# dream-faster/laplace-gnn-recommendation

Measured on AMD Instinct MI355X. Metric: positive-edges/sec (train step), higher is better.
Workload: dtype f32; 1 GPU; LightGCN train step, ONE synthetic bipartite graph 8000000x100000 users x items, 100000000 edges (seed 3, 64 user blocks), sharded by user over 1 GPU(s): 8000000 users / 100000000 edges per GPU, 3-layer D=128, global batch 131072 positive edges, on-device sampling, BPR + dense Adam; BASELINE.json configs[3]; parallelism=1 GPU

## Files before the change

### include/laplace_hip.h

```cpp
#ifndef LAPLACE_HIP_H
#define LAPLACE_HIP_H

#include <stddef.h>
#include <stdint.h>

#ifdef __cplusplus
extern "C" {
#endif

#define MI_ABI_VERSION 14

#define MI_ERR_BAD_ARG      (-1)
#define MI_ERR_TOO_LARGE    (-2)
#define MI_ERR_WORKSPACE    (-3)
#define MI_ERR_UNSUPPORTED  (-4)

typedef void* mi_stream_t;

int         mi_abi_version(void);
const char* mi_error_string(int code);

size_t mi_coo_to_csr_workspace_bytes(int64_t n_rows, int64_t nnz);
int    mi_coo_to_csr_i32(int64_t n_rows, int64_t n_cols, int64_t nnz,
                         const int64_t* row, const int64_t* col,
// ... 54 lines not shown
                               mi_spmm_plan_info* info, mi_stream_t stream);
int    mi_spmm_plan_fill(int64_t n_rows, const int32_t* rowptr, const mi_spmm_plan_info* info,
                         mi_spmm_plan* plan, void* ws, size_t ws_bytes, mi_stream_t stream);
size_t mi_spmm_plan_pack_workspace_bytes(int64_t n_launch);
int    mi_spmm_plan_pack_entries(const mi_spmm_plan* plan, int64_t nnz_long, const int32_t* col, const float* val,
                                 int32_t values_only, void* ws, size_t ws_bytes, mi_stream_t stream);
size_t mi_spmm_workspace_bytes(const mi_spmm_plan* plan, int64_t d);

int mi_spmm_csr_f32(int64_t n_rows, int64_t d,
                    const int32_t* rowptr, const int32_t* col, const float* val,
                    const float* X, int64_t ldx,
                    float* Y, int64_t ldy,
                    const float* addend, int64_t lda,
                    float* S, int64_t lds, float scale,
                    const mi_spmm_plan* plan, void* ws, size_t ws_bytes,
                    mi_stream_t stream);

typedef struct mi_adam_args {
    float*       p;  int64_t ldp;
    float*       m;
    float*       v;
    const float* reg_w;
    double       lr, beta1, beta2, eps;
    int64_t      step;
} mi_adam_args;

typedef struct mi_spmm_sweep {
    const int32_t* col;
    const float*   val;
    const int32_t* stream_ptr;
    const int32_t* slot_of;
    int32_t        n_streams;
    int32_t        n_slots;
    int32_t*       progress;
    int32_t        epoch;
    int32_t        slack;
} mi_spmm_sweep;

typedef struct mi_spmm_ex {
    const int32_t* x_map;
    const int32_t* addend_map;
    const int32_t* row_list;
    const int32_t* n_list_dev;
    int64_t        n_list;
    const mi_adam_args* adam;
    int32_t        parts;
    int32_t        hot_rows;
    const mi_spmm_sweep* sweep;
    int32_t        hot_base;
    int32_t        hot_threads;
    const uint32_t* x_bits;
    const int32_t* thin_rows;
    int32_t        n_thin;
} mi_spmm_ex;
#define MI_SPMM_SHORT_ROWS 1
#define MI_SPMM_SPLIT_ROWS 2

int mi_spmm_csr_ex_f32(int64_t n_rows, int64_t d,
                       const int32_t* rowptr, const int32_t* col, const float* val,
                       const float* X, int64_t ldx,
                       float* Y, int64_t ldy,
                       const float* addend, int64_t lda,
                       float* S, int64_t lds, float scale,
                       const mi_spmm_plan* plan, const mi_spmm_ex* ex,
                       void* ws, size_t ws_bytes, mi_stream_t stream);

int mi_map_live_bits_i32(int64_t n, const int32_t* map, uint32_t* bits, mi_stream_t stream);

int mi_gather_rows_f32(int64_t n_max, const int32_t* n_dev, const int32_t* begin_dev, int64_t d,
                       const int32_t* rows, int64_t row_offset, const float* src, int64_t ld_src,
                       float* dst, int64_t ld_dst, int32_t accumulate, float scale,
                       mi_stream_t stream);

int mi_scatter_rows_f32(int64_t n_max, const int32_t* n_dev, const int32_t* begin_dev, int64_t d,
                        const int32_t* rows, int64_t row_offset, const float* src, int64_t ld_src,
                        float* dst, int64_t ld_dst, mi_stream_t stream);

size_t mi_batch_nodes_workspace_bytes(int64_t n_nodes);
int    mi_batch_nodes_i32(int64_t batch, int64_t n_users, int64_t n_nodes,
                          const int64_t* users, const int64_t* pos, const int64_t* neg,
                          int32_t* gmap, int32_t* nodes, int32_t* count,
                          void* ws, size_t ws_bytes, mi_stream_t stream);

#define MI_SAMPLE_KEY_COLLISION 1
#define MI_SAMPLE_NO_SELF_LOOPS 2
int mi_csr_expand_rows(int64_t n_rows, const int32_t* rowptr, int32_t* row_of_edge,
                       int64_t nnz, mi_stream_t stream);
int mi_sample_bpr_batch(int64_t batch, int64_t nnz,
                        const int32_t* rowptr, const int32_t* col,
                        const int32_t* row_of_edge,
                        int64_t neg_range, int32_t quirk_user_rows, int32_t edges_in_order,
                        uint64_t seed, uint64_t step,
                        int64_t* users, int64_t* pos, int64_t* neg,
                        mi_stream_t stream);

size_t mi_bpr_workspace_bytes(int64_t batch);
int    mi_bpr_fwd_bwd_f32(int64_t batch, int64_t d, int64_t n_users,
                          const int64_t* users, const int64_t* pos, const int64_t* neg,
                          const float* final_emb, int64_t ldf,
                          const float* e0, int64_t lde,
                          float lambda, float g_scale, float reg_scale,
                          float* loss_out,
                          float* g_final, int64_t ldg,
                          float* reg_w,
                          const int32_t* node_map,
                          void* ws, size_t ws_bytes, mi_stream_t stream);
// ... 467 lines not shown
```

### laplace-gnn-recommendation_amd/_lib.py

```python
from __future__ import annotations

import ctypes
import os
from ctypes import POINTER, Structure, c_char_p, c_double, c_float, c_int32, c_int64, c_size_t, c_uint32, c_uint64, c_void_p

PKG_DIR = os.path.dirname(os.path.abspath(__file__))
LIB_PATH = os.environ.get("LAPLACE_HIP_LIB") or os.path.join(PKG_DIR, "liblaplace_hip.so")

MI_ABI_VERSION = 14
MI_SPMM_GROUP = 32


class MiError(RuntimeError):
    pass


class SpmmPlanStruct(Structure):
    _fields_ = [
        ("chunk", c_int32), ("n_long_rows", c_int32), ("n_items", c_int32), ("n_launch", c_int32),
        ("long_rows", c_void_p), ("item_ptr", c_void_p), ("items", c_void_p), ("long_index", c_void_p),
        ("band", c_int32), ("n_bands", c_int32),
        ("epos", c_void_p), ("ecol", c_void_p), ("eval", c_void_p),
    ]


class SpmmPlanInfo(Structure):
    _fields_ = [("n_long_rows", c_int64), ("n_items", c_int64), ("n_launch", c_int64), ("nnz_long", c_int64),
                ("chunk", c_int32), ("band", c_int32), ("n_bands", c_int32), ("queue_len", c_int32),
                ("queue_start", c_int32 * 9), ("keys_in_second", c_int32)]


class AdamArgs(Structure):
    _fields_ = [("p", c_void_p), ("ldp", c_int64), ("m", c_void_p), ("v", c_void_p), ("reg_w", c_void_p),
                ("lr", c_double), ("beta1", c_double), ("beta2", c_double), ("eps", c_double), ("step", c_int64)]


class SpmmSweepStruct(Structure):
    _fields_ = [("col", c_void_p), ("val", c_void_p), ("stream_ptr", c_void_p), ("slot_of", c_void_p),
                ("n_streams", c_int32), ("n_slots", c_int32), ("progress", c_void_p), ("epoch", c_int32), ("slack", c_int32)]


class SpmmExStruct(Structure):
    _fields_ = [("x_map", c_void_p), ("addend_map", c_void_p), ("row_list", c_void_p), ("n_list_dev", c_void_p),
                ("n_list", c_int64), ("adam", POINTER(AdamArgs)), ("parts", c_int32), ("hot_rows", c_int32),
                ("sweep", POINTER(SpmmSweepStruct)), ("hot_base", c_int32), ("hot_threads", c_int32),
                ("x_bits", c_void_p), ("thin_rows", c_void_p), ("n_thin", c_int32)]


MI_SPMM_SHORT_ROWS, MI_SPMM_SPLIT_ROWS = 1, 2
MI_ERR_UNSUPPORTED = -4
MI_ERR_BAD_ARG = -1
MI_ERR_TOO_LARGE = -2
MI_ERR_WORKSPACE = -3
MI_TOPK_ITEMS_PREPARED = 1
MI_RECENT_MAX_SLOTS = 16
MI_TOPK_MERGE_MAX_ENTRIES = 4096
MI_TOPK_PATH_MATERIALISED, MI_TOPK_PATH_ONE_PASS, MI_TOPK_PATH_FUSED, MI_TOPK_PATH_FUSED_DMA, MI_TOPK_PATH_PREFILTER = range(5)
MI_RANK_OBJECTIVES = {"reference": 0, "bpr": 1, "softmax": 2}
MI_RANK_MAX_NEG = 16
MI_COOC_WEIGHTINGS = {"count": 0, "cosine": 1}


class GemmProblem(Structure):
    _fields_ = [("trans_a", c_int32), ("trans_b", c_int32), ("m", c_int64), ("n", c_int64), ("k", c_int64),
                ("A", c_void_p), ("lda", c_int64), ("B", c_void_p), ("ldb", c_int64),
                ("k2", c_int64), ("A2", c_void_p), ("lda2", c_int64), ("B2", c_void_p), ("ldb2", c_int64),
                ("a_mask", c_void_p), ("bias", c_void_p), ("C", c_void_p), ("ldc", c_int64),
                ("accumulate", c_int32), ("act", c_int32)]


class SamplerDesc(Structure):
    _fields_ = [("batch", c_int32), ("n_hops", c_int32), ("num_neighbors", c_int32), ("k", c_int32),
                ("randomization", c_int32), ("max_pos", c_int32), ("max_neg", c_int32), ("reserved", c_int32),
                ("num_users", c_int64), ("num_articles", c_int64), ("num_edges", c_int64), ("id_max", c_int64),
                ("users_ptr", c_void_p), ("users_idx", c_void_p), ("articles_ptr", c_void_p), ("articles_idx", c_void_p),
                ("positive_edges_ratio", c_double), ("negative_edges_ratio", c_double), ("reject_min_entries", c_int64),
                ("cand_ptr", c_void_p), ("cand_idx", c_void_p)]


MI_SAMPLER_MAX_RELATIONS = 4


class SamplerRelation(Structure):
    _fields_ = [("rel_ptr", c_void_p), ("rel_idx", c_void_p), ("n_targets", c_int64)]


class SamplerRelationOut(Structure):
    _fields_ = [("t_ids", c_void_p), ("t_ptr", c_void_p), ("edge3", c_void_p), ("article_rowptr", c_void_p),
                ("article_col", c_void_p), ("t_rowptr", c_void_p), ("t_col", c_void_p), ("t_cursor", c_void_p)]


MI_RANKER_MAX_LAYERS, MI_RANKER_MAX_COLS, MI_RANKER_MAX_PARAMS = 4, 16, 48


class RankerConv(Structure):
    _fields_ = [("w_l", c_void_p), ("b_l", c_void_p), ("w_r", c_void_p), ("gw_l", c_void_p), ("gb_l", c_void_p), ("gw_r", c_void_p),
                ("c_src", c_int32), ("c_dst", c_int32), ("c_out", c_int32), ("reserved", c_int32)]


# ... 316 lines not shown
```

### laplace-gnn-recommendation_amd/csrc/spmm.hip

```cpp
#include "common.hpp"
#include "pairs.hpp"
#include <algorithm>
#include <rocprim/rocprim.hpp>

namespace {

#ifndef MI_SPMM_UNROLL
#define MI_SPMM_UNROLL 4
#endif
#ifndef MI_SPMM_UNROLL_ADAM
#define MI_SPMM_UNROLL_ADAM 8
#endif
#ifndef MI_SPMM_UNROLL_PAIR
#define MI_SPMM_UNROLL_PAIR 8
#endif
#ifndef MI_SPMM_ROWS_RPS
#define MI_SPMM_ROWS_RPS 1
#endif
#ifndef MI_SPMM_NT
#define MI_SPMM_NT 0
#endif
typedef float mi_f4v __attribute__((ext_vector_type(4)));
#ifndef MI_SPMM_SC1
#define MI_SPMM_SC1 6
#endif
template <int BIT>
__device__ __forceinline__ void mi_store4(float4* p, const float4& v, bool streaming) {
    if (((MI_SPMM_SC1 >> BIT) & 1) && streaming) {
        mi_f4v x = {v.x, v.y, v.z, v.w};
        asm volatile("global_store_dwordx4 %0, %1, off sc1\n\ts_nop 1" : : "v"(p), "v"(x) : "memory");
    } else if ((MI_SPMM_NT >> BIT) & 1) {
        mi_f4v x = {v.x, v.y, v.z, v.w};
        __builtin_nontemporal_store(x, reinterpret_cast<mi_f4v*>(p));
    } else {
        *p = v;
    }
}
template <int BIT>
__device__ __forceinline__ float4 mi_load4(const float4* p) {
    if ((MI_SPMM_NT >> BIT) & 1) {
        mi_f4v x = __builtin_nontemporal_load(reinterpret_cast<const mi_f4v*>(p));
        return make_float4(x.x, x.y, x.z, x.w);
    }
    return *p;
}
#ifndef MI_SPMM_FIXUP_UNROLL
#define MI_SPMM_FIXUP_UNROLL 32
#endif
constexpr int kWavesPerBlock = 4;
constexpr int kBlock = kWavesPerBlock * MI_WAVE;
constexpr int kPlanGroup = MI_SPMM_GROUP;

struct Epilogue {
    float4* Y;            int64_t ldy4;
    const float4* addend; int64_t lda4;
    float4* S;            int64_t lds4;
    float scale;
    bool streaming;
    float4* p;            int64_t ldp4;
    float4* m;
    float4* v;
    const float* reg_w;
    MiAdamConsts adam;
};

struct Ex {
    const int32_t* x_map;
    const int32_t* addend_map;
    const int32_t* row_list;
    const int32_t* n_list_dev;
    const int32_t* long_index;
    int32_t parts;
    int32_t hot_base, hot_rows, hot_threads;
    const uint32_t* x_bits;
    uint8_t* slot_live;
    const int32_t* thin_rows;
    int32_t n_thin;
};

template <int LPR>
__device__ __forceinline__ int wave_max_over_subgroups(int n) {
#pragma unroll
    for (int m = MI_WAVE / 2; m >= LPR; m >>= 1) n = max(n, __shfl_xor(n, m, MI_WAVE));
    return n;
}

template <int LPR, int VPL, int UNROLL, bool SPARSE>
__device__ __forceinline__ void subgroup_accumulate(const int32_t* __restrict__ col,
                                                    const float* __restrict__ val,
                                                    const float4* __restrict__ X4, int64_t ldx4, int d4,
                                                    int32_t beg, int n, int nmax, int li,
                                                    const int32_t* __restrict__ x_map, float4 (&acc)[VPL]) {
    static_assert(LPR % UNROLL == 0, "a batch of LPR entries is consumed UNROLL at a time");
#pragma unroll
    for (int v = 0; v < VPL; ++v) acc[v] = mi_f4_zero();
    for (int base = 0; base < nmax; base += LPR) {
        int32_t my_c = -1;
        float my_v = 0.f;
        if (base + li < n) {
            if (MI_SPMM_NT & 1) {
                my_c = __builtin_nontemporal_load(col + beg + base + li);
                my_v = __builtin_nontemporal_load(val + beg + base + li);
            } else {
                my_c = col[beg + base + li];
                my_v = val[beg + base + li];
            }
            if (SPARSE && x_map) my_c = x_map[my_c];
        }
        if (SPARSE && __ballot(my_c >= 0) == 0ull) continue;
        const int m = min(LPR, nmax - base);
        for (int j = 0; j < m; j += UNROLL) {
            float w[UNROLL];
            float4 x[UNROLL][VPL];
#pragma unroll
            for (int u = 0; u < UNROLL; ++u) {
                const int32_t c = __shfl(my_c, j + u, LPR);
                w[u] = __shfl(my_v, j + u, LPR);
                const bool ok = c >= 0;
                const float4* src = X4 + (int64_t)(ok ? c : 0) * ldx4;
#pragma unroll
                for (int v = 0; v < VPL; ++v) {
                    const int e = li + v * LPR;
                    x[u][v] = (ok && e < d4) ? src[e] : mi_f4_zero();
                }
                if (!ok) w[u] = 0.f;
            }
#pragma unroll
            for (int u = 0; u < UNROLL; ++u)
#pragma unroll
                for (int v = 0; v < VPL; ++v) mi_f4_fma(acc[v], w[u], x[u][v]);
// ... 84 lines not shown
        if (mine) {
            r = listed ? (int64_t)ex.row_list[i] : i;
            beg = rowptr[r];
            n = rowptr[r + 1] - beg;
            mine = n <= chunk;
        }
        if (kCoop && coop && mine && n > MI_SPMM_COOP_MIN) {
            if (li == 0) {
                const int q = atomicAdd(&coop_n, 1);
                coop_row[q] = r;
                coop_beg[q] = beg;
                coop_len[q] = n;
            }
            mine = false;
        }
        if (!mine) n = 0;
        const int nmax = wave_max_over_subgroups<LPR>(n);
        float4 a[VPL], acc[VPL];
        const int64_t ar = !mine ? -1 : (listed ? i : (ex.addend_map ? (int64_t)ex.addend_map[r] : r));
        load_addend<LPR, VPL>(ep, ar, d4, li, a);
        subgroup_accumulate<LPR, VPL, UNROLL, SPARSE>(col, val, X4, ldx4, d4, beg, n, nmax, li, ex.x_map, acc);
        if (mine) store_epilogue<LPR, VPL, ADAM>(ep, listed ? i : r, d4, li, acc, a);
    }
    if (kCoop && coop) {
        __syncthreads();
        const int n_long = coop_n;
        for (int q = 0; q < n_long; ++q) {
            const int32_t beg = coop_beg[q], len = coop_len[q];
            const int64_t r = coop_row[q];
            const int32_t per = (len + SG - 1) / SG;
            const int32_t b = min(sgi * per, len);
            const int n = min(per, len - b);
            const int nmax = wave_max_over_subgroups<LPR>(n);
            float4 acc[VPL];
            subgroup_accumulate<LPR, VPL, UNROLL, false>(col, val, X4, ldx4, d4, beg + b, n, nmax, li, nullptr, acc);
#pragma unroll
            for (int v = 0; v < VPL; ++v) coop_red[sgi][v][li] = acc[v];
            __syncthreads();
            if (sgi == 0) {
                float4 a[VPL];
                load_addend<LPR, VPL>(ep, ex.addend_map ? (int64_t)ex.addend_map[r] : r, d4, li, a);
#pragma unroll
                for (int v = 0; v < VPL; ++v) {
                    float4 t = coop_red[0][v][li];
                    for (int g = 1; g < SG; ++g) t = mi_f4_add(t, coop_red[g][v][li]);
                    acc[v] = t;
                }
                store_epilogue<LPR, VPL, ADAM>(ep, r, d4, li, acc, a);
            }
            __syncthreads();
        }
    }
}
template <int LPR, int VPL, int UNROLL, int RPS, bool SPARSE, bool ADAM>
__global__ __launch_bounds__(kBlock) void spmm_rows_kernel(int64_t n_out, int d4,
                                                           const int32_t* __restrict__ rowptr,
                                                           const int32_t* __restrict__ col,
                                                           const float* __restrict__ val,
                                                           const float4* __restrict__ X4, int64_t ldx4,
                                                           Epilogue ep, int32_t chunk, Ex ex, int32_t coop) {
    spmm_rows_body<LPR, VPL, UNROLL, RPS, SPARSE, ADAM>(blockIdx.x, gridDim.x, n_out, d4, rowptr, col, val, X4, ldx4, ep, chunk, ex, coop);
}
struct RowsSide {
    int64_t n_out; int d4;
    const int32_t* rowptr; const int32_t* col; const float* val;
    const float4* X4; int64_t ldx4;
    Epilogue ep;
};
template <int LPR, int UNROLL>
__global__ __launch_bounds__(kBlock) void spmm_rows_pair_kernel(RowsSide a, RowsSide b, unsigned split) {
    const bool first = blockIdx.x < split;
#define MI_PICK(f) (first ? a.f : b.f)
    Epilogue ep;
    ep.Y = MI_PICK(ep.Y);           ep.ldy4 = MI_PICK(ep.ldy4);
    ep.addend = MI_PICK(ep.addend); ep.lda4 = MI_PICK(ep.lda4);
    ep.S = MI_PICK(ep.S);           ep.lds4 = MI_PICK(ep.lds4);
    ep.scale = MI_PICK(ep.scale);
    ep.streaming = MI_PICK(ep.streaming);
    ep.p = nullptr; ep.ldp4 = 0; ep.m = nullptr; ep.v = nullptr; ep.reg_w = nullptr;
    ep.adam = MiAdamConsts{};
    const Ex ex = {nullptr, nullptr, nullptr, nullptr, nullptr, 0, 0, 0, 0, nullptr, nullptr, nullptr, 0};
    spmm_rows_body<LPR, 1, UNROLL, MI_SPMM_ROWS_RPS, false, false>(first ? blockIdx.x : blockIdx.x - split, first ? split : gridDim.x - split,
                                                                  MI_PICK(n_out), MI_PICK(d4), MI_PICK(rowptr), MI_PICK(col), MI_PICK(val),
                                                                  MI_PICK(X4), MI_PICK(ldx4), ep, INT32_MAX, ex, 1);
#undef MI_PICK
}


struct HotRows {
    int32_t base, n;
    int32_t row_bytes;
};

#define MI_HOT_ENTRY(U)                                                                                              \
    "v_subrev_u32_e32 %[t2], %[hbase], %[c" #U "]\n"       \
    "v_cmp_gt_u32_e32 vcc, %[hn], %[t2]\n"                 \
    "v_cmp_lt_i32_e64 %[m], -1, %[c" #U "]\n"              \
    "s_andn2_b64 %[m], %[m], vcc\n"                        \
    "s_and_b64 exec, %[save], vcc\n"                                                                                 \
    "v_mad_u32_u24 %[t2], %[t2], %[rowb], %[li16]\n"                                                                  \
    "ds_read_b128 %[x" #U "], %[t2]\n"                                                                                \
    "s_and_b64 exec, %[save], %[m]\n"                                                                                 \
    "v_mad_u64_u32 %[t01], vcc, %[c" #U "], %[ldb], %[xb]\n"                                                          \
    "global_load_dwordx4 %[x" #U "], %[t01], off\n"                                                                   \
    "s_mov_b64 exec, %[save]\n"

struct Prefetch {
    uint64_t rp;
    int32_t c;
    float v;
};

template <bool PRE>
__device__ __forceinline__ void hot_gather8(mi_f4v (&x)[8], const int32_t (&c)[8], const HotRows& hot, uint32_t ld_bytes,
// ... 910 lines not shown
    if (do_split && ex.n_thin > 0) {
        const int32_t waves = thin_waves();
        const int64_t n_slots = listed ? n_list : (int64_t)ex.n_thin;
        if (n_slots > 0)
            hipLaunchKernelGGL((spmm_thin_kernel<LPR, VPL, UNROLL_THIN, SPARSE, ADAM>),
                               dim3((unsigned)mi_ceil_div(n_slots, (int64_t)(kWavesPerBlock / waves))), dim3(kBlock), 0, s, n_slots,
                               waves, d4, rowptr, col, val, X4, ldx4, ep, ex);
    }
    const int64_t n_out = listed ? n_list : n_rows;
    bool short_done = false;
    if constexpr (!SPARSE && VPL == 1) {
        if (do_short && n_out > 0 && plan && ex.hot_rows != 0) {
            auto kern = spmm_rows_hot_kernel<LPR, UNROLL, ADAM>;
            static HotLaunch hl;
            const int thr_arg = ex.hot_threads & 0xFFF, waves_arg = ex.hot_threads >> 12;
            const int threads = thr_arg == 512 ? 512 : (thr_arg == 1024 ? 1024 : 256);
            const size_t row_bytes = (size_t)d4 * sizeof(float4);
            if (hl.state == 0) {
                hl.state = -1;
                hipDeviceProp_t prop;
                int dev = 0;
                if (hipGetDevice(&dev) == hipSuccess && hipGetDeviceProperties(&prop, dev) == hipSuccess) {
                    hl.cus = prop.multiProcessorCount;
                    hl.lds_cap = (size_t)prop.maxSharedMemoryPerMultiProcessor;
                    const size_t optin = hl.lds_cap > 1024 ? hl.lds_cap - 1024 : 0;
                    if (hl.cus > 0 && optin >= row_bytes &&
                        hipFuncSetAttribute(reinterpret_cast<const void*>(kern), hipFuncAttributeMaxDynamicSharedMemorySize,
                                            (int)optin) == hipSuccess)
                        hl.state = 1;
                }
            }
            if (hl.state == 1) {
                int wg_per_cu = std::max(1, (waves_arg > 0 ? waves_arg : MI_SPMM_HOT_WAVES) / (threads / MI_WAVE));
                const size_t share = (hl.lds_cap / (size_t)wg_per_cu) - 512;
                const int hot_n = (int)std::min<size_t>((size_t)std::max(ex.hot_rows, 0), share / row_bytes);
                const size_t lds = (size_t)hot_n * row_bytes;
                const int key = threads * 4 + (hot_n > 0 ? 1 : 0);
                if (hl.occ_key != key) {
                    int occ = 0;
                    if (hipOccupancyMaxActiveBlocksPerMultiprocessor(&occ, reinterpret_cast<const void*>(kern), threads, lds) != hipSuccess)
                        occ = 0;
                    hl.occ_key = key;
                    hl.occ = occ;
                }
                wg_per_cu = std::min(wg_per_cu, hl.occ);
                if (wg_per_cu > 0) {
                    hipLaunchKernelGGL(kern, dim3((unsigned)(hl.cus * wg_per_cu)), dim3(threads), lds, s, n_rows, d4, rowptr, col,
                                       val, X4, ldx4, ep, chunk, ex, ex.hot_base, hot_n);
                    short_done = true;
                }
            }
        }
    }
    if (do_short && n_out > 0 && !short_done) {
        dim3 gr((unsigned)mi_ceil_div(n_out, SG * ROWS_RPS));
        if (MI_SPMM_XCD_RANGES && !listed) gr.x = (gr.x + 7u) / 8u * 8u;
        hipLaunchKernelGGL((spmm_rows_kernel<LPR, VPL, UNROLL_ROWS, ROWS_RPS, SPARSE, ADAM>), gr, dim3(kBlock), 0, s, n_out, d4,
                           rowptr, col, val, X4, ldx4, ep, chunk, ex, plan ? 0 : 1);
    }
    if (do_split && plan && plan->n_long_rows > 0) {
        const int64_t nf = listed ? n_list : (int64_t)plan->n_long_rows;
        Ex exf = ex;
        if (!xmap_form) exf.slot_live = nullptr;
        if (nf > 0)
            hipLaunchKernelGGL((spmm_fixup_kernel<LPR, VPL, SPARSE, ADAM>), dim3((unsigned)nf), dim3(kBlock), 0, s,
                               (int32_t)nf, d4, plan->long_rows, plan->item_ptr, partial, ep, exf);
    }
    return mi_launch_status();
}

template <int LPR, int VPL>
int launch_spmm(int64_t n_rows, int d4, const int32_t* rowptr, const int32_t* col, const float* val,
                const float4* X4, int64_t ldx4, const Epilogue& ep, const mi_spmm_plan* plan,
                float4* partial, const Ex& ex, int64_t n_list, hipStream_t s, const mi_spmm_sweep* sweep) {
    const bool sparse = ex.x_map || ex.row_list;
#define MI_SPMM_GO(SP, AD) \
    return launch_spmm_mode<LPR, VPL, SP, AD>(n_rows, d4, rowptr, col, val, X4, ldx4, ep, plan, partial, ex, n_list, s, sweep)
    if (ep.p) {
        if (sparse) MI_SPMM_GO(true, true);
        MI_SPMM_GO(false, true);
    }
    if (sparse) MI_SPMM_GO(true, false);
    MI_SPMM_GO(false, false);
#undef MI_SPMM_GO
}

}

static inline bool n_cols_ok(const mi_spmm_sweep*) { return true; }

extern "C" {

size_t mi_spmm_plan_workspace_bytes(int64_t n_rows, int64_t nnz) {
    if (n_rows < 0 || nnz < 0) return 0;
    const size_t n1 = (size_t)n_rows + 1, z = (size_t)(nnz > 0 ? nnz : 1);
    return 4 * mi_align_up(n1 * 4, 256) + 256 + plan_tmp_bytes(nnz > n_rows + 1 ? nnz : n_rows + 1) +
           2 * mi_align_up(n1 * 4, 256) + 3 * mi_align_up(z * 4, 256) + 2 * mi_align_up(z * 8, 256);
}

int mi_spmm_plan_count(int64_t n_rows, int64_t n_cols, const int32_t* rowptr, const int32_t* col,
                       int32_t chunk, int32_t band, void* ws, size_t ws_bytes, mi_spmm_plan_info* info,
                       mi_stream_t stream) {
    return mi_spmm_plan_count_range(n_rows, n_cols, rowptr, col, chunk, INT32_MAX, band, ws, ws_bytes, info, stream);
}

int mi_spmm_plan_count_range(int64_t n_rows, int64_t n_cols, const int32_t* rowptr, const int32_t* col,
// ... 143 lines not shown
    constexpr int kPerBlock = 256 / 32;
    hipLaunchKernelGGL(plan_pack_kernel, dim3((unsigned)mi_ceil_div(n, (int64_t)kPerBlock)), dim3(256), 0, s, n,
                       reinterpret_cast<const int4*>(plan->items), plan->epos, (int32_t)nnz_long, col, val,
                       values_only ? nullptr : plan->ecol, plan->eval);
    return mi_launch_status();
}

size_t mi_spmm_workspace_bytes(const mi_spmm_plan* plan, int64_t d) {
    if (!plan || plan->n_items <= 0) return 0;
    return mi_align_up((size_t)plan->n_items * (size_t)d * sizeof(float), 256) + mi_align_up((size_t)plan->n_items, 256);
}

int mi_map_live_bits_i32(int64_t n, const int32_t* map, uint32_t* bits, mi_stream_t stream) {
    MI_CHECK_ARG(n >= 0 && (n == 0 || (map && bits)));
    if (n == 0) return 0;
    hipLaunchKernelGGL(map_live_bits_kernel, dim3((unsigned)mi_ceil_div(n, (int64_t)kBlock)), dim3(kBlock), 0, (hipStream_t)stream, n, map,
                       bits);
    return mi_launch_status();
}

int mi_spmm_csr_ex_f32(int64_t n_rows, int64_t d, const int32_t* rowptr, const int32_t* col,
                       const float* val, const float* X, int64_t ldx, float* Y, int64_t ldy,
                       const float* addend, int64_t lda, float* S, int64_t lds, float scale,
                       const mi_spmm_plan* plan, const mi_spmm_ex* exh, void* ws, size_t ws_bytes,
                       mi_stream_t stream) {
    MI_CHECK_ARG(n_rows >= 0 && d > 0 && rowptr);
    if (n_rows == 0) return 0;
    if (d % 4 != 0 || d > 512) return MI_ERR_UNSUPPORTED;
    if (n_rows >= INT32_MAX) return MI_ERR_TOO_LARGE;
    const mi_adam_args* adam = exh ? exh->adam : nullptr;
    MI_CHECK_ARG(X && (Y || S || adam));
    MI_CHECK_ARG(ldx % 4 == 0 && ldx >= d && mi_aligned16(X));
    MI_CHECK_ARG(!Y || (ldy % 4 == 0 && ldy >= d && mi_aligned16(Y) && Y != X));
    MI_CHECK_ARG(!S || (lds % 4 == 0 && lds >= d && mi_aligned16(S) && S != X));
    MI_CHECK_ARG(!addend || (lda % 4 == 0 && lda >= d && mi_aligned16(addend)));
    Ex ex = {nullptr, nullptr, nullptr, nullptr, nullptr, MI_SPMM_SHORT_ROWS | MI_SPMM_SPLIT_ROWS, 0, 0, 0, nullptr, nullptr, nullptr, 0};
    int64_t n_list = 0;
    if (exh) {
        ex.x_map = exh->x_map;
        ex.addend_map = exh->addend_map;
        ex.row_list = exh->row_list;
        ex.n_list_dev = exh->n_list_dev;
        n_list = exh->n_list;
        if (exh->parts) {
            MI_CHECK_ARG((exh->parts & ~(MI_SPMM_SHORT_ROWS | MI_SPMM_SPLIT_ROWS)) == 0);
            ex.parts = exh->parts;
        }
        if (!ex.x_map && !ex.row_list && d <= 256) {
            MI_CHECK_ARG(exh->hot_base >= 0 && exh->hot_threads >= 0);
            ex.hot_base = exh->hot_base;
            ex.hot_rows = exh->hot_rows;
            ex.hot_threads = exh->hot_threads;
        }
        if (exh->n_thin > 0) {
            MI_CHECK_ARG(plan && exh->thin_rows);
            ex.thin_rows = exh->thin_rows;
            ex.n_thin = exh->n_thin;
        }
        if (ex.row_list) {
            MI_CHECK_ARG(n_list >= 0 && !ex.addend_map);
            if (n_list == 0) return 0;
            if (plan && (plan->n_long_rows > 0 || ex.n_thin > 0)) {
                MI_CHECK_ARG(plan->long_index);
                ex.long_index = plan->long_index;
            }
        }
    }
    const mi_spmm_sweep* sweep = (exh && plan && plan->n_items > 0) ? exh->sweep : nullptr;
    if (sweep) {
        MI_CHECK_ARG(sweep->col && sweep->val && sweep->stream_ptr && sweep->slot_of);
        MI_CHECK_ARG(sweep->n_streams > 0 && sweep->n_streams % 32 == 0 && sweep->n_streams <= 32 * 32);
        MI_CHECK_ARG(sweep->n_slots > 0 && n_cols_ok(sweep) &&
                     (plan->items ? plan->n_items > 8 * sweep->n_slots : plan->n_items == 8 * sweep->n_slots));
        MI_CHECK_ARG(sweep->slack >= 0);
        if (d > 128) return MI_ERR_UNSUPPORTED;
    }
    float4* partial = nullptr;
    if (plan && plan->n_items > 0) {
        const int64_t own_items = (int64_t)plan->n_items - (sweep ? 8 * (int64_t)sweep->n_slots : 0);
        MI_CHECK_ARG(plan->item_ptr && plan->long_rows && (sweep || plan->items));
        MI_CHECK_ARG(!plan->items || plan->n_launch >= own_items);
        MI_CHECK_ARG(!plan->items || plan->band == 0 || plan->n_launch % (8 * kPlanGroup) == 0);
        MI_CHECK_ARG(!plan->epos || (plan->items && plan->ecol && plan->eval));
        if (!ws || ws_bytes < mi_spmm_workspace_bytes(plan, d)) return MI_ERR_WORKSPACE;
        MI_CHECK_ARG(mi_aligned16(ws) && (!plan->items || mi_aligned16(plan->items)));
        partial = reinterpret_cast<float4*>(ws);
        if (exh && exh->x_bits && ex.x_map && plan->items && plan->epos && !sweep && !ex.row_list) {
            ex.x_bits = exh->x_bits;
            ex.slot_live = reinterpret_cast<uint8_t*>(ws) + mi_align_up((size_t)plan->n_items * (size_t)d * sizeof(float), 256);
        }
    }
    Epilogue ep;
    ep.Y = reinterpret_cast<float4*>(Y);                 ep.ldy4 = ldy / 4;
    ep.addend = reinterpret_cast<const float4*>(addend); ep.lda4 = lda / 4;
    ep.S = reinterpret_cast<float4*>(S);                 ep.lds4 = lds / 4;
    ep.scale = scale;
    ep.streaming = (size_t)n_rows * (size_t)d * sizeof(float) >= ((size_t)64 << 20);
    ep.p = nullptr; ep.ldp4 = 0; ep.m = nullptr; ep.v = nullptr; ep.reg_w = nullptr;
    ep.adam = MiAdamConsts{};
    if (adam) {
        MI_CHECK_ARG(!ex.row_list && adam->p && adam->m && adam->v && adam->step >= 1);
        MI_CHECK_ARG(adam->ldp % 4 == 0 && adam->ldp >= d && mi_aligned16(adam->p) && mi_aligned16(adam->m) &&
                     mi_aligned16(adam->v));
        MI_CHECK_ARG(adam->p != X && adam->p != Y && adam->p != S && adam->p != addend);
        ep.p = reinterpret_cast<float4*>(adam->p);
        ep.ldp4 = adam->ldp / 4;
// ... 71 lines not shown
```

### laplace-gnn-recommendation_amd/ops.py

```python
from __future__ import annotations

import ctypes
import itertools
import os
from os import environ as _os_environ
from dataclasses import dataclass, field
from typing import Optional, Tuple

import torch as t
from torch import Tensor

from . import _lib
from ._lib import SpmmExStruct, SpmmPlanStruct, SpmmSweepStruct, check

DEFAULT_CHUNK = 256
DEFAULT_BAND = int(_os_environ.get("LAPLACE_SPMM_BAND", 16384))
MIN_BANDED_COLS = 131072
THIN_PER_BAND = int(_os_environ.get("LAPLACE_SPMM_THIN", 2))

SPMM_EVENTS = None

SPMM_TWO_STREAMS = int(os.environ.get("LAPLACE_SPMM_TWO_STREAMS", "1") or 0)
PACK_ENTRIES = os.environ.get("LAPLACE_SPMM_PACK", "1") != "0"
X_RARE_BITS = os.environ.get("LAPLACE_X_RARE", "1") != "0"
# ... 37 lines not shown
def _rows_ok(x: Tensor, name: str) -> int:
    try:
        if x.dtype is t.float32 and x.is_cuda and x.dim() == 2:
            (r, c), (s0, s1) = x.shape, x.stride()
            if c <= 1 or s1 == 1:
                return s0 if r > 1 else max(c, s0)
    except AttributeError:
        pass
    _need(x, t.float32, name, contiguous=False)
    if x.dim() == 2 and x.shape[0] == 0:
        return max(int(x.shape[1]), 1)
    if x.dim() != 2 or (x.shape[1] > 1 and x.stride(1) != 1):
        raise ValueError(f"{name}: expected a row-major 2-D matrix, got shape {tuple(x.shape)} strides {x.stride()}")
    return x.stride(0) if x.shape[0] > 1 else max(x.shape[1], x.stride(0))


def _ws(nbytes: int, device) -> Tensor:
    return t.empty(max(int(nbytes), 256), dtype=t.uint8, device=device)


_WS_CACHE = {}


def _ws_reused(nbytes: int, device) -> Tensor:
    dev = t.device(device) if not isinstance(device, int) else t.device("cuda", device)
    key = (dev.index if dev.index is not None else t.cuda.current_device(), _stream())
    cur = _WS_CACHE.get(key)
    if cur is None or cur.numel() < nbytes:
        cur = t.empty(max(int(nbytes) * 2, 1 << 20), dtype=t.uint8, device=dev)
        _WS_CACHE[key] = cur
    return cur


_VAL_GEN = itertools.count(1)


@dataclass
class SpmmPlan:
    struct: SpmmPlanStruct
    long_rows: Optional[Tensor]
    item_ptr: Optional[Tensor]
    items: Optional[Tensor]
    long_index: Optional[Tensor] = None
    partial: dict = field(default_factory=dict)
    sweep: Optional[SpmmSweepStruct] = None
    sweep_t: tuple = ()
    wide: Optional["SpmmPlan"] = None
    packed: tuple = ()
    sweep_src: Optional[Tensor] = None
    values_of: tuple = ()
    nnz_long: int = 0
    thin_rows: Optional[Tensor] = None
    thin_max: int = 0

    @property
    def n_thin_rows(self) -> int:
        return int(self.thin_rows.numel()) if self.thin_rows is not None else 0

    @property
    def n_split_rows(self) -> int:
        return int(self.struct.n_long_rows)

    @property
    def n_long_rows(self) -> int:
        return int(self.struct.n_long_rows) + self.n_thin_rows

    @property
    def n_items(self) -> int:
        return int(self.struct.n_items)


@dataclass
class DeviceCSR:
    n_rows: int
    n_cols: int
    rowptr: Tensor
    col: Tensor
    val: Optional[Tensor] = None
    perm: Optional[Tensor] = None
    plan: Optional[SpmmPlan] = None
    hot: Optional[Tuple[int, int]] = None

    _val_gen = 0

    def __setattr__(self, name, value):
        if name == "val" and "val" in self.__dict__:
            object.__setattr__(self, "_val_gen", next(_VAL_GEN))
        object.__setattr__(self, name, value)

    def invalidate_values(self) -> None:
        object.__setattr__(self, "_val_gen", next(_VAL_GEN))

    @property
    def nnz(self) -> int:
        return int(self.col.numel())

    @property
    def device(self):
        return self.rowptr.device


def coo_to_csr(row: Tensor, col: Tensor, n_rows: int, n_cols: int, want_perm: bool = True) -> DeviceCSR:
    _need(row, t.int64, "row")
    _need(col, t.int64, "col")
    if row.shape != col.shape or row.dim() != 1:
        raise ValueError("row/col must be 1-D tensors of equal length")
# ... 15 lines not shown
    col_t = t.empty(a.nnz, dtype=t.int32, device=dev)
    perm_t = t.empty(a.nnz, dtype=t.int32, device=dev)
    L = _lib.lib()
    ws = _ws(L.mi_csr_transpose_workspace_bytes(a.n_rows, a.nnz), dev)
    check(L.mi_csr_transpose_i32(a.n_rows, a.n_cols, a.nnz, _ptr(a.rowptr), _ptr(a.col), _ptr(rowptr_t),
                                 _ptr(col_t), _ptr(perm_t), ws.data_ptr(), ws.numel(), _stream()),
          "mi_csr_transpose_i32")
    val_t = gather_f32(a.val, perm_t) if a.val is not None else None
    return DeviceCSR(a.n_cols, a.n_rows, rowptr_t, col_t, val_t, perm_t)


def gather_f32(src: Tensor, idx: Tensor) -> Tensor:
    _need(src, t.float32, "src")
    _need(idx, t.int32, "idx")
    out = t.empty(idx.numel(), dtype=t.float32, device=src.device)
    check(_lib.lib().mi_gather_f32(idx.numel(), _ptr(src), _ptr(idx), _ptr(out), _stream()), "mi_gather_f32")
    return out


def gcn_norm(a: DeviceCSR, val_in: Optional[Tensor] = None) -> Tuple[Tensor, Tensor]:
    if a.n_rows != a.n_cols:
        raise ValueError("gcn_norm needs a square adjacency")
    if val_in is not None:
        _need(val_in, t.float32, "val_in")
    val = t.empty(a.nnz, dtype=t.float32, device=a.device)
    dis = t.empty(a.n_rows, dtype=t.float32, device=a.device)
    check(_lib.lib().mi_gcn_norm_csr_f32(a.n_rows, a.nnz, _ptr(a.rowptr), _ptr(a.col), _ptr(val_in),
                                         _ptr(val), _ptr(dis), _stream()), "mi_gcn_norm_csr_f32")
    return val, dis


def scale_csr(a: DeviceCSR, val_in: Optional[Tensor] = None, row_scale: Optional[Tensor] = None,
              col_scale: Optional[Tensor] = None) -> Tensor:
    for n, x in (("val_in", val_in), ("row_scale", row_scale), ("col_scale", col_scale)):
        if x is not None:
            _need(x, t.float32, n)
    if row_scale is not None and row_scale.numel() != a.n_rows:
        raise ValueError("row_scale must have one entry per row")
    if col_scale is not None and col_scale.numel() != a.n_cols:
        raise ValueError("col_scale must have one entry per column")
    out = t.empty(a.nnz, dtype=t.float32, device=a.device)
    check(_lib.lib().mi_scale_csr_f32(a.n_rows, a.nnz, _ptr(a.rowptr), _ptr(a.col), _ptr(val_in), _ptr(row_scale),
                                      _ptr(col_scale), _ptr(out), _stream()), "mi_scale_csr_f32")
    return out


def row_slice(a: DeviceCSR, r0: int, r1: int) -> DeviceCSR:
    return DeviceCSR(r1 - r0, a.n_cols, a.rowptr[r0:r1 + 1], a.col, a.val, None, None, a.hot)


PERSISTENT_ROWS = _os_environ.get("LAPLACE_PERSISTENT_ROWS", "0") == "1"
HOT_ROWS = int(_os_environ.get("LAPLACE_HOT_ROWS", 304))
HOT_THREADS = int(_os_environ.get("LAPLACE_HOT_THREADS", 0))


def hot_item_rows(num_users: int, num_items: int) -> Optional[Tuple[int, int]]:
    if HOT_ROWS <= 0 or num_items <= 0:
        return None
    return (int(num_users), int(min(HOT_ROWS, num_items)))


SWEEP_BAND = 2048
SWEEP_STREAMS = 1024
SWEEP_MIN_BANDS = 64
SWEEP_PACE = 0


def build_sweep_plan(a: DeviceCSR, chunk: int = DEFAULT_CHUNK, band: int = SWEEP_BAND,
                     n_streams: int = SWEEP_STREAMS, min_deg: Optional[int] = None) -> Optional[SpmmPlan]:
    import heapq
    if a.val is None or a.nnz == 0 or a.n_cols >= (1 << 27) or a.n_cols < SWEEP_MIN_BANDS * band:
        return None
    dev = a.device
    deg = (a.rowptr[1:] - a.rowptr[:-1]).to(t.int64)

    def slots_for(ch: int):
        rows = t.nonzero(deg > ch).view(-1)
        if rows.numel() == 0:
            return rows, [], 0, [], 0
        host = deg[rows].cpu().tolist()
        tot = sum(host)
        target = max(ch, tot // (3 * n_streams))
        pp = [max(1, -(-d // target)) for d in host]
        return rows, host, tot, pp, sum(pp)

    long_rows, dl_host, total, parts, n_slots = slots_for(chunk if min_deg is None else max(int(min_deg), chunk))
    if long_rows.numel() == 0:
        return None
    if n_slots > 8 * n_streams:
        return None
    n_long = int(long_rows.numel())
    dl = deg[long_rows]
    loads = []
    slot_base = [0] * (n_long + 1)
    for i, (d, p) in enumerate(zip(dl_host, parts)):
        slot_base[i + 1] = slot_base[i] + p
        loads += [(d / p, slot_base[i] + j) for j in range(p)]
    loads.sort(key=lambda z: (-z[0], z[1]))
    heap = [(0.0, k, 0) for k in range(n_streams)]
    heapq.heapify(heap)
    owner = [0] * n_slots
    qidx = [0] * n_slots
    slot_of = [-1] * (8 * n_streams)
    full = []
    for w, sid in loads:
        while True:
# ... 263 lines not shown
        _need(m_, t.float32, "adam.m")
        _need(v_, t.float32, "adam.v")
        if tuple(p_.shape) != (a.n_rows, d) or m_.shape != p_.shape or v_.shape != p_.shape:
            raise ValueError(f"adam.p/m/v must be [{a.n_rows}, {d}]")
        rw = adam.get("reg_w")
        if rw is not None:
            _need(rw, t.float32, "adam.reg_w")
        adam_args = _lib.AdamArgs(p_.data_ptr(), ldp, m_.data_ptr(), v_.data_ptr(), _ptr(rw), float(adam["lr"]),
                                  float(adam.get("beta1", 0.9)), float(adam.get("beta2", 0.999)),
                                  float(adam.get("eps", 1e-8)), int(adam["step"]))
    ldy = _rows_ok(Y, "Y") if Y is not None else 0
    lda = _rows_ok(addend, "addend") if addend is not None else 0
    lds = _rows_ok(S, "S") if S is not None else 0
    if a.plan is None and (a.nnz >= PLAN_MIN_NNZ or row_list is not None):
        a.plan = build_spmm_plan(a)
    plan = a.plan
    if plan is not None and plan.sweep is not None and d > 128:
        if plan.wide is None:
            plan.wide = build_spmm_plan(a, chunk=int(plan.struct.chunk), sweep=False, thin_max=0)
        plan = plan.wide
    L = _lib.lib()
    if plan is not None and plan.values_of:
        _sync_plan_values(a, plan)
    ws_ptr, ws_bytes = None, 0
    if plan is not None and plan.n_items > 0:
        if d not in plan.partial:
            plan.partial[d] = _ws(L.mi_spmm_workspace_bytes(ctypes.byref(plan.struct), d), a.device)
        ws_ptr, ws_bytes = plan.partial[d].data_ptr(), plan.partial[d].numel()
    col_ptr = _ptr(a.col) if a.nnz else a.rowptr.data_ptr()
    val_ptr = _ptr(a.val) if a.nnz else a.rowptr.data_ptr()
    ev = None
    if SPMM_EVENTS is not None:
        ev = (t.cuda.Event(enable_timing=True), t.cuda.Event(enable_timing=True))
        ev[0].record()
    sweep = plan.sweep if (plan is not None and plan.sweep is not None) else None
    hot_base, hot_rows = 0, (-1 if PERSISTENT_ROWS else 0)
    if (a.hot is not None and plan is not None and x_map is None and row_list is None and d <= 256 and HOT_ROWS > 0
            and PERSISTENT_ROWS):
        hot_base, hot_rows = int(a.hot[0]), int(a.hot[1])
        if hot_rows == 0:
            hot_rows = -1
        if hot_base < 0 or hot_rows < -1 or hot_base + max(hot_rows, 0) > X.shape[0]:
            raise ValueError(f"hot rows [{hot_base}, {hot_base + hot_rows}) lie outside X ({X.shape[0]} rows)")

    x_bits = None
    if (x_rare and X_RARE_BITS and x_map is not None and row_list is None and sweep is None and plan is not None
            and plan.n_items > 0):
        x_bits = getattr(a, "_x_bits", None)
        if x_bits is None:
            x_bits = a._x_bits = t.empty((a.n_cols + 31) // 32, dtype=t.int32, device=a.device)
        check(L.mi_map_live_bits_i32(a.n_cols, _ptr(x_map), _ptr(x_bits), _stream()), "mi_map_live_bits_i32")

    n_thin = plan.n_thin_rows if plan is not None else 0

    def launch(parts: int, stream: int) -> None:
        exs = None
        if (x_map is not None or addend_map is not None or row_list is not None or adam_args is not None or parts
                or sweep is not None or hot_rows != 0 or HOT_THREADS or n_thin):
            exs = SpmmExStruct(_ptr(x_map), _ptr(addend_map), _ptr(row_list), _ptr(n_list_dev),
                               row_list.numel() if row_list is not None else 0,
                               ctypes.pointer(adam_args) if adam_args is not None else None, parts, hot_rows,
                               ctypes.pointer(sweep) if sweep is not None else None, hot_base, HOT_THREADS, _ptr(x_bits),
                               _ptr(plan.thin_rows) if n_thin else None, n_thin)
        check(L.mi_spmm_csr_ex_f32(a.n_rows, d, _ptr(a.rowptr), col_ptr, val_ptr, X.data_ptr(), ldx,
                                   _ptr(Y), ldy, _ptr(addend), lda, _ptr(S), lds, float(scale),
                                   ctypes.byref(plan.struct) if plan is not None else None,
                                   ctypes.byref(exs) if exs is not None else None, ws_ptr, ws_bytes,
                                   stream), "mi_spmm_csr_ex_f32")

    if SPMM_TWO_STREAMS and plan is not None and (plan.n_items > 0 or n_thin > 0):
        cur = t.cuda.current_stream()
        side = _side_stream(a.device)
        side.wait_stream(cur)
        if SPMM_TWO_STREAMS == 2:
            launch(_lib.MI_SPMM_SPLIT_ROWS, cur.cuda_stream)
            launch(_lib.MI_SPMM_SHORT_ROWS, side.cuda_stream)
        else:
            launch(_lib.MI_SPMM_SHORT_ROWS, side.cuda_stream)
            launch(_lib.MI_SPMM_SPLIT_ROWS, cur.cuda_stream)
        cur.wait_stream(side)
    else:
        launch(0, _stream())
    if ev is not None:
        ev[1].record()
        kind = "sparse" if (x_map is not None or row_list is not None) else ("dense_adam" if adam is not None else "dense")
        SPMM_EVENTS.append((ev[0], ev[1], kind, None, a.n_rows, a))


def expand_rows(a: DeviceCSR) -> Tensor:
    out = t.empty(a.nnz, dtype=t.int32, device=a.device)
    check(_lib.lib().mi_csr_expand_rows(a.n_rows, _ptr(a.rowptr), _ptr(out), a.nnz, _stream()),
          "mi_csr_expand_rows")
    return out


def check_n_neg(n_neg: int) -> int:
    if not isinstance(n_neg, int) or isinstance(n_neg, bool) or not 1 <= n_neg <= _lib.MI_RANK_MAX_NEG:
        raise ValueError(f"n_neg must be an integer in 1..{_lib.MI_RANK_MAX_NEG}, got {n_neg!r}")
    return n_neg


def rank_objective_code(objective: str) -> int:
    if objective not in _lib.MI_RANK_OBJECTIVES:
        raise ValueError(f"objective must be one of {sorted(_lib.MI_RANK_OBJECTIVES)}, got {objective!r}")
    return _lib.MI_RANK_OBJECTIVES[objective]


def sample_bpr_batch(r: DeviceCSR, row_of_edge: Tensor, batch: int, neg_range: int, seed: int, step: int,
                     quirk: bool = False, out: Optional[Tuple[Tensor, Tensor, Tensor]] = None,
                     edges_in_order: bool = False, no_self_loops: bool = False, n_neg: int = 1
                     ) -> Tuple[Tensor, Tensor, Tensor]:
    check_n_neg(n_neg)
    if r.nnz == 0:
        raise ValueError("cannot sample from an empty edge set")
    if neg_range <= 0:
        raise ValueError("neg_range must be positive")
# ... 631 lines not shown
```

Before: 2.795 million positive-edges/s.

## Add column-sliced SpMM row kernel with XCD-aligned slices and shared-memory CSR staging

```diff
diff --git a/include/laplace_hip.h b/include/laplace_hip.h
--- a/include/laplace_hip.h
+++ b/include/laplace_hip.h
@@ -130,6 +130,8 @@
     const uint32_t* x_bits;
     const int32_t* thin_rows;
     int32_t        n_thin;
+    int32_t        row_slices;
+    int32_t        slice_rows;
 } mi_spmm_ex;
 #define MI_SPMM_SHORT_ROWS 1
 #define MI_SPMM_SPLIT_ROWS 2
diff --git a/laplace-gnn-recommendation_amd/_lib.py b/laplace-gnn-recommendation_amd/_lib.py
--- a/laplace-gnn-recommendation_amd/_lib.py
+++ b/laplace-gnn-recommendation_amd/_lib.py
@@ -44,7 +44,8 @@
     _fields_ = [("x_map", c_void_p), ("addend_map", c_void_p), ("row_list", c_void_p), ("n_list_dev", c_void_p),
                 ("n_list", c_int64), ("adam", POINTER(AdamArgs)), ("parts", c_int32), ("hot_rows", c_int32),
                 ("sweep", POINTER(SpmmSweepStruct)), ("hot_base", c_int32), ("hot_threads", c_int32),
-                ("x_bits", c_void_p), ("thin_rows", c_void_p), ("n_thin", c_int32)]
+                ("x_bits", c_void_p), ("thin_rows", c_void_p), ("n_thin", c_int32), ("row_slices", c_int32),
+                ("slice_rows", c_int32)]
 
 
 MI_SPMM_SHORT_ROWS, MI_SPMM_SPLIT_ROWS = 1, 2
diff --git a/laplace-gnn-recommendation_amd/csrc/spmm.hip b/laplace-gnn-recommendation_amd/csrc/spmm.hip
--- a/laplace-gnn-recommendation_amd/csrc/spmm.hip
+++ b/laplace-gnn-recommendation_amd/csrc/spmm.hip
@@ -76,6 +76,8 @@
     uint8_t* slot_live;
     const int32_t* thin_rows;
     int32_t n_thin;
+    int32_t row_slices;
+    int32_t slice_rows;
 };
 
 template <int LPR>
@@ -266,14 +268,168 @@
         }
     }
 }
-template <int LPR, int VPL, int UNROLL, int RPS, bool SPARSE, bool ADAM>
+#ifndef MI_SPMM_SLICE_TILE
+#define MI_SPMM_SLICE_TILE 128
+#endif
+#ifndef MI_SPMM_SLICE_CAP
+#define MI_SPMM_SLICE_CAP 2048
+#endif
+#ifndef MI_SPMM_SLICE_UNROLL
+#define MI_SPMM_SLICE_UNROLL 4
+#endif
+constexpr int kSliceTile = MI_SPMM_SLICE_TILE;
+constexpr int kSliceCap = MI_SPMM_SLICE_CAP;
+static_assert(kSliceTile <= kBlock && kSliceTile <= 65535, "one thread ranks one row of the tile");
+
+template <int LPR, int UNROLL, bool SPARSE, bool ADAM, int SL>
+__device__ __forceinline__ void spmm_rows_sliced_body(int64_t n_rows, int d4,
+                                                      const int32_t* __restrict__ rowptr,
+                                                      const int32_t* __restrict__ col,
+                                                      const float* __restrict__ val,
+                                                      const float4* __restrict__ X4, int64_t ldx4,
+                                                      const Epilogue& ep, int32_t chunk, const Ex& ex) {
+    constexpr int NB = MI_WAVE / LPR, SG = NB * kWavesPerBlock, PER = 8 / SL;
+    __shared__ int32_t s_rp[kSliceTile + 1];
+    __shared__ int32_t s_len[kSliceTile];
+    __shared__ uint16_t s_order[kSliceTile];
+    __shared__ int32_t s_col[kSliceCap];
+    __shared__ float s_val[kSliceCap];
+    const int xcd = blockIdx.x & 7;
+    const int slice = xcd % SL;
+    const int64_t tile = (int64_t)(blockIdx.x >> 3) * PER + xcd / SL;
+    const int64_t t0 = tile * kSliceTile;
+    if (t0 >= n_rows) return;
+    const int nt = (int)min((int64_t)kSliceTile, n_rows - t0);
+    const int w = d4 / SL;
+    const int lane = mi_lane();
+    const int li = lane % LPR;
+    const int sgi = (threadIdx.x / MI_WAVE) * NB + lane / LPR;
+    const bool lane_on = li < w;
+    const int e = slice * w + li;
+    for (int i = threadIdx.x; i <= nt; i += kBlock) s_rp[i] = rowptr[t0 + i];
+    __syncthreads();
+    for (int i = threadIdx.x; i < nt; i += kBlock) {
+        const int n = s_rp[i + 1] - s_rp[i];
+        s_len[i] = (n <= chunk) ? n : 0;
+    }
+    __syncthreads();
+    int r0 = 0;
+    while (r0 < nt) {
+        if (s_rp[r0 + 1] - s_rp[r0] > chunk) {
+            ++r0;
+            continue;
+        }
+        const int32_t g0 = s_rp[r0];
+        int lo = r0 + 1, hi = nt;
+        while (lo < hi) {
+            const int mid = (lo + hi + 1) >> 1;
+            if (s_rp[mid] - g0 <= kSliceCap) lo = mid; else hi = mid - 1;
+        }
+        const int r1 = lo, m = r1 - r0;
+        const int span = s_rp[r1] - g0;
+        for (int p = threadIdx.x; p < span; p += kBlock) {
+            int32_t c = col[g0 + p];
+            if (SPARSE && ex.x_map) c = ex.x_map[c];
+            s_col[p] = c;
+            s_val[p] = val[g0 + p];
+        }
+        if ((int)threadIdx.x < m) {
+            const int i = threadIdx.x, key = s_len[r0 + i];
+            int rank = 0;
+            for (int j = 0; j < m; ++j) {
+                const int kj = s_len[r0 + j];
+                rank += (kj > key || (kj == key && j < i)) ? 1 : 0;
+            }
+            s_order[rank] = (uint16_t)i;
+        }
+        __syncthreads();
+        float wv[UNROLL];
+        float4 xv[UNROLL], a;
+        int pos = sgi, off = 0, n = 0;
+        int64_t r = 0;
+        bool mine = false;
+        auto open_row = [&]() {
+            n = 0;
+            mine = false;
+            if (pos < m) {
+                const int i = r0 + s_order[pos];
+                n = s_len[i];
+                off = s_rp[i] - g0;
+                r = t0 + i;
+                mine = lane_on && s_rp[i + 1] - s_rp[i] <= chunk;
+            }
+            a = mi_f4_zero();
+            if (mine && (ep.S || ep.p) && ep.addend) {
+                const int64_t ar = ex.addend_map ? (int64_t)ex.addend_map[r] : r;
+                if (ar >= 0) a = mi_load4<3>(ep.addend + ar * ep.lda4 + e);
+            }
+#pragma unroll
+            for (int u = 0; u < UNROLL; ++u) {
+                const bool in = u < n;
+                const int32_t c = in ? s_col[off + u] : -1;
+                wv[u] = (in && c >= 0) ? s_val[off + u] : 0.f;
+                xv[u] = (c >= 0 && lane_on) ? X4[(int64_t)c * ldx4 + e] : mi_f4_zero();
+            }
+        };
+        open_row();
+        while (pos < m) {
+            float4 acc = mi_f4_zero();
+#pragma unroll
+            for (int u = 0; u < UNROLL; ++u) mi_f4_fma(acc, wv[u], xv[u]);
+            for (int k = UNROLL; k < n; k += UNROLL) {
+#pragma unroll
+                for (int u = 0; u < UNROLL; ++u) {
+                    const bool in = k + u < n;
+                    const int32_t c = in ? s_col[off + k + u] : -1;
+                    wv[u] = (in && c >= 0) ? s_val[off + k + u] : 0.f;
+                    xv[u] = (c >= 0 && lane_on) ? X4[(int64_t)c * ldx4 + e] : mi_f4_zero();
+                }
+#pragma unroll
+                for (int u = 0; u < UNROLL; ++u) mi_f4_fma(acc, wv[u], xv[u]);
+            }
+            const int64_t rs = r;
+            const float4 as = a;
+            const bool mine_s = mine;
+            pos += SG;
+            if constexpr (!ADAM) open_row();
+            if (mine_s) {
+                if (ep.Y) mi_store4<2>(ep.Y + rs * ep.ldy4 + e, acc, ep.streaming);
+                if (ep.S || ADAM) {
+                    float4 o;
+                    o.x = ep.scale * (as.x + acc.x);
+                    o.y = ep.scale * (as.y + acc.y);
+                    o.z = ep.scale * (as.z + acc.z);
+                    o.w = ep.scale * (as.w + acc.w);
+                    if (ep.S) mi_store4<2>(ep.S + rs * ep.lds4 + e, o, ep.streaming);
+                    if (ADAM) {
+                        const float rw = ep.reg_w ? ep.reg_w[rs] : 0.f;
+                        const int64_t i = rs * d4 + e;
+                        float4 pp = ep.p[rs * ep.ldp4 + e], mm = ep.m[i], vv = ep.v[i];
+                        mi_adam_update4(pp, o, mm, vv, ep.reg_w != nullptr, rw, ep.adam);
+                        ep.p[rs * ep.ldp4 + e] = pp;
+                        ep.m[i] = mm;
+                        ep.v[i] = vv;
+                    }
+                }
+            }
+            if constexpr (ADAM) open_row();
+        }
+        __syncthreads();
+        r0 = r1;
+    }
+}
+
+template <int LPR, int VPL, int UNROLL, int RPS, bool SPARSE, bool ADAM, int SL = 0>
 __global__ __launch_bounds__(kBlock) void spmm_rows_kernel(int64_t n_out, int d4,
                                                            const int32_t* __restrict__ rowptr,
                                                            const int32_t* __restrict__ col,
                                                            const float* __restrict__ val,
                                                            const float4* __restrict__ X4, int64_t ldx4,
                                                            Epilogue ep, int32_t chunk, Ex ex, int32_t coop) {
-    spmm_rows_body<LPR, VPL, UNROLL, RPS, SPARSE, ADAM>(blockIdx.x, gridDim.x, n_out, d4, rowptr, col, val, X4, ldx4, ep, chunk, ex, coop);
+    if constexpr (SL > 1)
+        spmm_rows_sliced_body<LPR, UNROLL, SPARSE, ADAM, SL>(n_out, d4, rowptr, col, val, X4, ldx4, ep, chunk, ex);
+    else
+        spmm_rows_body<LPR, VPL, UNROLL, RPS, SPARSE, ADAM>(blockIdx.x, gridDim.x, n_out, d4, rowptr, col, val, X4, ldx4, ep, chunk, ex, coop);
 }
 struct RowsSide {
     int64_t n_out; int d4;
@@ -1290,6 +1446,40 @@
             }
         }
     }
+    if constexpr (VPL == 1) {
+        const int sl = ex.row_slices;
+        if (do_short && n_out > 0 && !short_done && plan && !listed && (sl == 2 || sl == 4) && d4 % sl == 0 &&
+            chunk <= kSliceCap && (!SPARSE || ex.x_map)) {
+            const int64_t n_sl = ex.slice_rows > 0 ? std::min<int64_t>(ex.slice_rows, n_out) : n_out;
+            const int64_t tiles = mi_ceil_div(n_sl, kSliceTile);
+            const dim3 gs((unsigned)(mi_ceil_div(tiles, 8 / sl) * 8));
+            if (sl == 2)
+                hipLaunchKernelGGL((spmm_rows_kernel<LPR / 2, 1, MI_SPMM_SLICE_UNROLL, 1, SPARSE, ADAM, 2>), gs, dim3(kBlock), 0, s, n_sl, d4,
+                                   rowptr, col, val, X4, ldx4, ep, chunk, ex, 0);
+            else
+                hipLaunchKernelGGL((spmm_rows_kernel<LPR / 4, 1, MI_SPMM_SLICE_UNROLL, 1, SPARSE, ADAM, 4>), gs, dim3(kBlock), 0, s, n_sl, d4,
+                                   rowptr, col, val, X4, ldx4, ep, chunk, ex, 0);
+            if (n_sl < n_out) {
+                Epilogue er = ep;
+                Ex exr = ex;
+                if (er.Y) er.Y += n_sl * er.ldy4;
+                if (er.S) er.S += n_sl * er.lds4;
+                if (exr.addend_map) exr.addend_map += n_sl;
+                else if (er.addend) er.addend += n_sl * er.lda4;
+                if (er.p) {
+                    er.p += n_sl * er.ldp4;
+                    er.m += n_sl * d4;
+                    er.v += n_sl * d4;
+                    if (er.reg_w) er.reg_w += n_sl;
+                }
+                const int64_t n_rest = n_out - n_sl;
+                hipLaunchKernelGGL((spmm_rows_kernel<LPR, VPL, UNROLL_ROWS, ROWS_RPS, SPARSE, ADAM>),
+                                   dim3((unsigned)mi_ceil_div(n_rest, SG * ROWS_RPS)), dim3(kBlock), 0, s, n_rest, d4, rowptr + n_sl,
+                                   col, val, X4, ldx4, er, chunk, exr, 0);
+            }
+            short_done = true;
+        }
+    }
     if (do_short && n_out > 0 && !short_done) {
         dim3 gr((unsigned)mi_ceil_div(n_out, SG * ROWS_RPS));
         if (MI_SPMM_XCD_RANGES && !listed) gr.x = (gr.x + 7u) / 8u * 8u;
@@ -1539,6 +1729,10 @@
             ex.hot_rows = exh->hot_rows;
             ex.hot_threads = exh->hot_threads;
         }
+        MI_CHECK_ARG(exh->row_slices == 0 || exh->row_slices == 1 || exh->row_slices == 2 || exh->row_slices == 4);
+        MI_CHECK_ARG(exh->slice_rows >= 0);
+        ex.row_slices = exh->row_slices;
+        ex.slice_rows = exh->slice_rows;
         if (exh->n_thin > 0) {
             MI_CHECK_ARG(plan && exh->thin_rows);
             ex.thin_rows = exh->thin_rows;
diff --git a/laplace-gnn-recommendation_amd/ops.py b/laplace-gnn-recommendation_amd/ops.py
--- a/laplace-gnn-recommendation_amd/ops.py
+++ b/laplace-gnn-recommendation_amd/ops.py
@@ -113,6 +113,7 @@
     nnz_long: int = 0
     thin_rows: Optional[Tensor] = None
     thin_max: int = 0
+    slice_reuse: dict = field(default_factory=dict)
 
     @property
     def n_thin_rows(self) -> int:
@@ -234,6 +235,21 @@
 PERSISTENT_ROWS = _os_environ.get("LAPLACE_PERSISTENT_ROWS", "0") == "1"
 HOT_ROWS = int(_os_environ.get("LAPLACE_HOT_ROWS", 304))
 HOT_THREADS = int(_os_environ.get("LAPLACE_HOT_THREADS", 0))
+
+
+ROW_SLICES = int(_os_environ.get("LAPLACE_SPMM_ROW_SLICES", 2))
+ROW_SLICES_FORMS = int(_os_environ.get("LAPLACE_SPMM_ROW_SLICES_FORMS", 1))
+ROW_SLICES_MIN_REUSE = float(_os_environ.get("LAPLACE_SPMM_ROW_SLICES_MIN_REUSE", 400))
+
+
+def _row_slices_pay(a: "DeviceCSR", plan: "SpmmPlan", slice_rows: int) -> bool:
+    if ROW_SLICES_MIN_REUSE <= 0:
+        return True
+    if slice_rows not in plan.slice_reuse:
+        nnz = int(a.rowptr[slice_rows]) if slice_rows else a.nnz
+        cols = a.n_cols - (min(int(a.hot[0]), a.n_cols) if slice_rows else 0)
+        plan.slice_reuse[slice_rows] = nnz / max(cols, 1)
+    return plan.slice_reuse[slice_rows] >= ROW_SLICES_MIN_REUSE
 
 
 def hot_item_rows(num_users: int, num_items: int) -> Optional[Tuple[int, int]]:
@@ -603,16 +619,22 @@
         check(L.mi_map_live_bits_i32(a.n_cols, _ptr(x_map), _ptr(x_bits), _stream()), "mi_map_live_bits_i32")
 
     n_thin = plan.n_thin_rows if plan is not None else 0
+    form = 4 if x_map is not None else (2 if adam is not None else 1)
+    row_slices = ROW_SLICES if (ROW_SLICES in (2, 4) and a.hot is not None and plan is not None and row_list is None
+                                and (ROW_SLICES_FORMS & form)) else 0
+    slice_rows = max(0, min(int(a.hot[0]), a.n_rows)) if row_slices else 0
+    if row_slices and not _row_slices_pay(a, plan, slice_rows):
+        row_slices = slice_rows = 0
 
     def launch(parts: int, stream: int) -> None:
         exs = None
         if (x_map is not None or addend_map is not None or row_list is not None or adam_args is not None or parts
-                or sweep is not None or hot_rows != 0 or HOT_THREADS or n_thin):
+                or sweep is not None or hot_rows != 0 or HOT_THREADS or n_thin or row_slices):
             exs = SpmmExStruct(_ptr(x_map), _ptr(addend_map), _ptr(row_list), _ptr(n_list_dev),
                                row_list.numel() if row_list is not None else 0,
                                ctypes.pointer(adam_args) if adam_args is not None else None, parts, hot_rows,
                                ctypes.pointer(sweep) if sweep is not None else None, hot_base, HOT_THREADS, _ptr(x_bits),
-                               _ptr(plan.thin_rows) if n_thin else None, n_thin)
+                               _ptr(plan.thin_rows) if n_thin else None, n_thin, row_slices, slice_rows)
         check(L.mi_spmm_csr_ex_f32(a.n_rows, d, _ptr(a.rowptr), col_ptr, val_ptr, X.data_ptr(), ldx,
                                    _ptr(Y), ldy, _ptr(addend), lda, _ptr(S), lds, float(scale),
                                    ctypes.byref(plan.struct) if plan is not None else None,
```

Measured after the change: 2.824 million positive-edges/s (median of 6 runs). 1.1% higher.
